# Shuijing725/CrowdNav_Prediction_AttnGraph

Hardware: NVIDIA H100
Metric: env_steps_per_s_ppo_rollout (higher is better)
Workload: dtype f32

## Files before the change

### crowdnav_prediction_attngraph_b200/csrc/cn_gemm_tc.cu

```cuda
#include "cn_gemm_tc.h"

__global__ void cn_split_f16_kernel(const float* __restrict__ src, float scale, __half* __restrict__ hi,
                                    __half* __restrict__ lo, size_t count) {
  const size_t i = (size_t)blockIdx.x * blockDim.x + threadIdx.x;
  if (i >= count) return;
  const float x = fminf(fmaxf(src[i] * scale, -65504.0f), 65504.0f);
  const __half h = __float2half_rn(x);
  hi[i] = h;
  lo[i] = __float2half_rn(x - __half2float(h));
}

namespace {

typedef CUresult (*EncodeFn)(CUtensorMap*, CUtensorMapDataType, cuuint32_t, void*, const cuuint64_t*, const cuuint64_t*,
                             const cuuint32_t*, const cuuint32_t*, CUtensorMapInterleave, CUtensorMapSwizzle,
                             CUtensorMapL2promotion, CUtensorMapFloatOOBfill);

EncodeFn get_encode() {
  static EncodeFn fn = nullptr;
  if (!fn) {
    void* sym = nullptr;
    cudaDriverEntryPointQueryResult qres;
    if (cudaGetDriverEntryPoint("cuTensorMapEncodeTiled", &sym, cudaEnableDefault, &qres) == cudaSuccess &&
        qres == cudaDriverEntryPointSuccess)
// ... 61 lines not shown
  cuuint64_t gstride[1] = {(cuuint64_t)pitch * esize};
  cuuint32_t box[2] = {(cuuint32_t)(128 / esize), 64};
  cuuint32_t estr[2] = {1, 1};
  CUresult r = enc(&s->map, esize == 4 ? CU_TENSOR_MAP_DATA_TYPE_FLOAT32 : CU_TENSOR_MAP_DATA_TYPE_FLOAT16, 2,
                   const_cast<void*>(ptr), gdim, gstride, box, estr, CU_TENSOR_MAP_INTERLEAVE_NONE,
                   CU_TENSOR_MAP_SWIZZLE_128B, CU_TENSOR_MAP_L2_PROMOTION_NONE, CU_TENSOR_MAP_FLOAT_OOB_FILL_NONE);
  if (r != CUDA_SUCCESS) return cn_set_error("cuTensorMapEncodeTiled(store) failed (%d) rows=%d cols=%d", (int)r, rows, cols);
  s->rows = rows; s->cols = cols;
  return 0;
}

int tc_alloc(CnLaunchCtx* c, TcMat& t, int rows, int K, int box_rows, int box_k) {
  int rc = halloc16(c, &t.hi, (size_t)rows * K);
  if (!rc) rc = halloc16(c, &t.lo, (size_t)rows * K);
  t.pitch = K; t.box_k = box_k;
  if (!rc) rc = make_map(&t.mh, t.hi, rows, K, box_rows, K, box_k);
  if (!rc) rc = make_map(&t.ml, t.lo, rows, K, box_rows, K, box_k);
  if (!rc) rc = tc_store_maps(t, rows, K);
  return rc;
}

int tc_view(TcMat& v, const TcMat& src, int col0, int rows, int K, int box_rows) {
  v.hi = src.hi + col0; v.lo = src.lo + col0; v.pitch = src.pitch; v.box_k = src.box_k;
  int rc = make_map(&v.mh, v.hi, rows, K, box_rows, src.pitch, src.box_k);
  if (!rc) rc = make_map(&v.ml, v.lo, rows, K, box_rows, src.pitch, src.box_k);
  if (!rc) rc = tc_store_maps(v, rows, K);
  return rc;
}

void split16(CnLaunchCtx* c, cudaStream_t st, const float* src, float scale, __half* hi, __half* lo, size_t count) {
  cn_split_f16_kernel<<<(unsigned)((count + 255) / 256), 256, 0, st>>>(src, scale, hi, lo, count);
  c->launches += 1;
}

int tc_set_attrs() {
  cudaError_t e = cudaSuccess;
  for (int act = CN_ACT_NONE; act <= CN_ACT_TANH; ++act)
    for (int out = TC_OUT_F32; out <= TC_OUT_BOTH; ++out) {
      if (e == cudaSuccess)
        e = cudaFuncSetAttribute(tc_kernel<256>(act, out), cudaFuncAttributeMaxDynamicSharedMemorySize, TcCfg<256>::kSmemBytes);
      if (e == cudaSuccess)
        e = cudaFuncSetAttribute(tc_kernel<64>(act, out), cudaFuncAttributeMaxDynamicSharedMemorySize, TcCfg<64>::kSmemBytes);
    }
  if (e == cudaSuccess)
    e = cudaFuncSetAttribute(cn_gemm_tc_kernel<64, true>, cudaFuncAttributeMaxDynamicSharedMemorySize, TcCfg<64>::kSmemBytes);
  if (e == cudaSuccess)
    e = cudaFuncSetAttribute(cn_gemm_tc_kernel<256, false, CN_ACT_NONE, TC_OUT_GRU>,
                             cudaFuncAttributeMaxDynamicSharedMemorySize, TcCfg<256>::kSmemBytes);
  if (e != cudaSuccess) return cn_set_error("cudaFuncSetAttribute(tc): %s", cudaGetErrorString(e));
  return 0;
}

void gemm_tc(CnLaunchCtx* c, cudaStream_t st, const TcMat& A, const TcMat& B, int M, int N, int K, int bn, const float* bias,
             int act, const TcOut& o, const int* m_ptr, int act_lo, int act_hi, const int* m0_ptr) {
  TcEpilogue ep;
  memset(&ep, 0, sizeof(ep));
  ep.bias = bias; ep.inv_scale = 1.0f / 64.0f; ep.act = act; ep.act_lo = act_lo; ep.act_hi = act_hi;
  ep.c32 = o.c32; ep.ldc = o.ldc; ep.out_hi = o.oh; ep.out_lo = o.ol; ep.ldh = o.ldh; ep.m_ptr = m_ptr; ep.m0_ptr = m0_ptr;
  {
    static const int nostore = (getenv("CN_DBG_NOSTORE") && getenv("CN_DBG_NOSTORE")[0] == '1') ? 1 : 0;
    ep.dbg_nostore = nostore;
  }
  if (A.box_k != tc_box_k(bn) || B.box_k != tc_box_k(bn)) {
    if (!c->launch_error) {
      c->launch_error = true;
      cn_set_error("gemm_tc in stage '%s': operand boxes %d / %d wide, the BN = %d instance loads %d",
                   c->cur_stage ? c->cur_stage : "?", A.box_k, B.box_k, bn, tc_box_k(bn));
    }
    return;
  }
  const int out_kind = (o.c32 ? TC_OUT_F32 : 0) | (o.oh ? TC_OUT_F16 : 0);
  if (act < CN_ACT_NONE || act > CN_ACT_TANH || !out_kind) {
    if (!c->launch_error) {
      c->launch_error = true;
      cn_set_error("gemm_tc in stage '%s': activation %d / no output", c->cur_stage ? c->cur_stage : "?", act);
    }
    return;
  }
#ifdef CN_GEMM_TRACE
  ep.trace = g_tc_trace; ep.trace_cap = g_tc_trace_cap;
#endif
  static const CUtensorMap no_map = {};
  const CUtensorMap *mc = &no_map, *mh = &no_map, *ml = &no_map;
  if (bn == 256) {
    auto fits = [&](const TcStoreMap* s) { return s && s->rows == M && s->cols == N; };
    const bool ok = (!o.c32 || fits(o.sc)) && (!o.oh || (fits(o.sh) && fits(o.sl)));
    if (!ok) {
      if (!c->launch_error) {
        c->launch_error = true;
        cn_set_error("gemm_tc in stage '%s': a BN = 256 output needs a TMA store map of [%d x %d] (16-byte-aligned "
                     "base, row pitch a multiple of 16 bytes)", c->cur_stage ? c->cur_stage : "?", M, N);
      }
      return;
    }
    if (o.c32) mc = &o.sc->map;
    if (o.oh) { mh = &o.sh->map; ml = &o.sl->map; }
  }
  const int tiles = (N / bn) * ((M + TC_BM - 1) / TC_BM);
  dim3 grid(tiles < c->num_sms ? tiles : c->num_sms);
  if (bn == 256)
    launch_k(c, tc_kernel<256>(act, out_kind), grid, dim3(TC_THREADS), TcCfg<256>::kSmemBytes, st, A.mh, A.ml, B.mh, B.ml, M, N, K, ep,
             *mc, *mh, *ml);
  else
    launch_k(c, tc_kernel<64>(act, out_kind), grid, dim3(TC_THREADS), TcCfg<64>::kSmemBytes, st, A.mh, A.ml, B.mh, B.ml, M, N, K, ep,
             *mc, *mh, *ml);
}

void gemm_tc_gru(CnLaunchCtx* c, cudaStream_t st, const TcMat& A, const TcMat& B, int M, const float* bias,
                 const float* h_in, const float* mask, float* h_out, int group, int pitch, int off, __half* oh, __half* ol,
                 int ldh) {
  const int N = 4 * 256, K = 64 + 256;
// ... 102 lines not shown
```

### crowdnav_prediction_attngraph_b200/csrc/cn_gemm_tc.cuh

```cuda
#pragma once
#include <cuda.h>
#include <cuda_fp16.h>
#include <cuda_runtime.h>
#include <stdint.h>

#include "cn_launch.cuh"

#define TC_BM 128
#define TC_BK 64
#define TC_CONSUMER_WARPS 8
#define TC_THREADS (128 + 32 * TC_CONSUMER_WARPS)

template <int BN>
struct TcCfg {
  static constexpr int kBK = (BN >= 256) ? 32 : TC_BK;
  static constexpr int kSwizzle = 2 * kBK;
  static constexpr int kStages = 4;
  static constexpr int kATile = TC_BM * kBK * 2;
  static constexpr int kBTile = BN * kBK * 2;
  static constexpr int kStageBytes = 2 * kATile + 2 * kBTile;
  static constexpr int kStoreBoxes = (BN >= 256) ? 2 : 0;
  static constexpr int kBoxBytes = 64 * 128;
  static constexpr int kStagingBytes = 2 * kStoreBoxes * kBoxBytes;
  static constexpr int kSmemBytes = kStages * kStageBytes + kStagingBytes + 256  + 1024 ;
};

struct TcEpilogue {
  const float* bias;
  float inv_scale;
  int act;
  int act_lo, act_hi;
  float* c32;
  int ldc;
  __half* out_hi;
  __half* out_lo;
  int ldh;
  const int* m_ptr;
  int dbg_nostore;
  const int* m0_ptr;
  const float* inv_scale_a;
  const float* inv_scale_b;
  int ksplit;
  const float* gru_h;
  const float* gru_mask;
  int gru_group, gru_pitch, gru_off;
#ifdef CN_GEMM_TRACE
  unsigned long long* trace;
  int trace_cap;
#endif
};

#ifdef CN_GEMM_TRACE
#define TC_TRACE_REC 7
#define TC_TRACE_WAIT_CLK 100
#endif

enum { TC_OUT_F32 = 1, TC_OUT_F16 = 2, TC_OUT_BOTH = 3, TC_OUT_GRU = 4 };

#ifdef CN_GEMM_TRACE
#define TC_TRACE(...) __VA_ARGS__
#else
#define TC_TRACE(...)
#endif

namespace tc {

__device__ __forceinline__ uint32_t smem_u32(const void* p) { return (uint32_t)__cvta_generic_to_shared(p); }

__device__ __forceinline__ void mbar_init(uint32_t bar, uint32_t count) {
  asm volatile("mbarrier.init.shared::cta.b64 [%0], %1;" ::"r"(bar), "r"(count));
}
__device__ __forceinline__ void mbar_expect_tx(uint32_t bar, uint32_t bytes) {
  asm volatile("mbarrier.arrive.expect_tx.shared::cta.b64 _, [%0], %1;" ::"r"(bar), "r"(bytes) : "memory");
}
__device__ __forceinline__ void mbar_arrive(uint32_t bar) {
  asm volatile("mbarrier.arrive.shared::cta.b64 _, [%0];" ::"r"(bar) : "memory");
}
__device__ __forceinline__ void mbar_wait(uint32_t bar, uint32_t parity) {
  uint32_t ok;
  do {
    asm volatile(
        "{\n"
        ".reg .pred p;\n"
        "mbarrier.try_wait.parity.shared::cta.b64 p, [%1], %2;\n"
        "selp.u32 %0, 1, 0, p;\n"
        "}\n" : "=r"(ok) : "r"(bar), "r"(parity) : "memory");
  } while (!ok);
}
#ifdef CN_GEMM_TRACE
__device__ __forceinline__ uint32_t mbar_wait_polls(uint32_t bar, uint32_t parity) {
  uint32_t ok, n = 0;
  while (true) {
// ... 351 lines not shown
  constexpr int TC_STAGE_BYTES = TcCfg<BN>::kStageBytes;
  constexpr bool kTmaStore = !PROMOTE && BN == 256 && OUT != TC_OUT_GRU;
  static_assert(OUT != TC_OUT_GRU || (BN == 256 && !PROMOTE), "the GRU epilogue reads four 64-column gate blocks");
  static_assert(!PROMOTE || BK == 64, "PROMOTE sums 64-wide k-blocks");
  static_assert(!kTmaStore || TcCfg<BN>::kStoreBoxes > 0, "BN = 256 stages its output");
  extern __shared__ uint8_t tc_smem_raw[];
  const uint32_t raw = tc::smem_u32(tc_smem_raw);
  const uint32_t base = (raw + 1023u) & ~1023u;
  const uint32_t staging = base + TC_STAGES * TC_STAGE_BYTES;
  const uint32_t bar_base = staging + TcCfg<BN>::kStagingBytes;
  const uint32_t bar_full = bar_base, bar_empty = bar_base + 64;

  const int warp = threadIdx.x >> 5, lane = threadIdx.x & 31, wg = warp >> 2;
  const int num_kb = K / BK;

  if (threadIdx.x == 0) {
    for (int s = 0; s < TC_STAGES; ++s) {
      tc::mbar_init(bar_full + 8 * s, 1);
      tc::mbar_init(bar_empty + 8 * s, TC_CONSUMER_WARPS);
    }
    asm volatile("fence.mbarrier_init.release.cluster;" ::: "memory");
    asm volatile("prefetch.tensormap [%0];" ::"l"(&map_ahi) : "memory");
    asm volatile("prefetch.tensormap [%0];" ::"l"(&map_alo) : "memory");
    asm volatile("prefetch.tensormap [%0];" ::"l"(&map_bhi) : "memory");
    asm volatile("prefetch.tensormap [%0];" ::"l"(&map_blo) : "memory");
    if constexpr (kTmaStore) {
      if constexpr ((OUT & TC_OUT_F32) != 0) asm volatile("prefetch.tensormap [%0];" ::"l"(&map_c) : "memory");
      if constexpr ((OUT & TC_OUT_F16) != 0) {
        asm volatile("prefetch.tensormap [%0];" ::"l"(&map_oh) : "memory");
        asm volatile("prefetch.tensormap [%0];" ::"l"(&map_ol) : "memory");
      }
    }
  }
  __syncthreads();
  cn_pdl_wait();
  const int m_ext = M;
  if (ep.m_ptr) { const int mc = *ep.m_ptr; M = mc < M ? mc : M; }
  int m_lo = ep.m0_ptr ? *ep.m0_ptr : 0;
  if (m_lo > M) m_lo = M;
  const int n_ntiles = N / BN;
  const int n_mn = ((M - m_lo + TC_BM - 1) / TC_BM) * n_ntiles;
  const int ksplit = (PROMOTE && ep.ksplit > 1) ? ep.ksplit : 1;
  const int kb_per = (num_kb + ksplit - 1) / ksplit;
  const int n_tiles = n_mn * ksplit;

  if (wg == 0) {
    tc::setmaxnreg_dec<40>();
    if (threadIdx.x == 0) {
      uint32_t it = 0;
      for (int tile = blockIdx.x; tile < n_tiles; tile += gridDim.x) {
        const int mn = tile % n_mn, ks = tile / n_mn;
        const int m0 = m_lo + (mn / n_ntiles) * TC_BM, n0 = (mn % n_ntiles) * BN;
        const int kb0 = ks * kb_per, kb1 = (kb0 + kb_per < num_kb) ? kb0 + kb_per : num_kb;
        for (int kb = kb0; kb < kb1; ++kb, ++it) {
          const uint32_t s = it % TC_STAGES, ph = (it / TC_STAGES) & 1u;
          tc::mbar_wait(bar_empty + 8 * s, ph ^ 1u);
          const uint32_t full = bar_full + 8 * s;
          tc::mbar_expect_tx(full, TC_STAGE_BYTES);
          const uint32_t st = base + s * TC_STAGE_BYTES;
          tc::tma_load_2d(st, &map_ahi, full, kb * BK, m0);
          tc::tma_load_2d(st + TC_A_TILE_BYTES, &map_alo, full, kb * BK, m0);
          tc::tma_load_2d(st + 2 * TC_A_TILE_BYTES, &map_bhi, full, kb * BK, n0);
          tc::tma_load_2d(st + 2 * TC_A_TILE_BYTES + TC_B_TILE_BYTES, &map_blo, full, kb * BK, n0);
        }
      }
    }
    return;
  }
  tc::setmaxnreg_inc<232>();
  float inv_scale = ep.inv_scale;
  if (ep.inv_scale_a) inv_scale *= __ldg(ep.inv_scale_a);
  if (ep.inv_scale_b) inv_scale *= __ldg(ep.inv_scale_b);
  const int half = wg - 1;
  const int wr = 16 * (warp & 3) + (lane >> 2);
  const int cq = 2 * (lane & 3);
  uint32_t it = 0;
  TcStaging sg;
  sg.base = staging + half * TcCfg<BN>::kStoreBoxes * TcCfg<BN>::kBoxBytes;
  sg.box = 0; sg.leader = (threadIdx.x & 127) == 0; sg.bar_id = wg;
  TC_TRACE(sg.waits = 0; sg.wait_clk = 0;)
  TC_TRACE(const bool tr = ep.trace && warp == 4 && lane == 0; int tr_n = 0;)
  for (int tile = blockIdx.x; tile < n_tiles; tile += gridDim.x) {
    const int mn = tile % n_mn, ks = tile / n_mn;
    const int m0 = m_lo + (mn / n_ntiles) * TC_BM, n0 = (mn % n_ntiles) * BN;
    const int kb0 = ks * kb_per, kb1 = (kb0 + kb_per < num_kb) ? kb0 + kb_per : num_kb;
    TC_TRACE(const uint64_t t_tile = tc::globaltimer(); uint64_t t_first = 0; uint32_t polls = 0;)
    float acc[BN / 2];
    float sum[PROMOTE ? BN / 2 : 1];
    if constexpr (PROMOTE) {
#pragma unroll
      for (int i = 0; i < BN / 2; ++i) sum[i] = 0.0f;
    }
    uint32_t prev = 0;
    for (int kb = kb0; kb < kb1; ++kb, ++it) {
      const uint32_t s = it % TC_STAGES, ph = (it / TC_STAGES) & 1u;
#ifdef CN_GEMM_TRACE
      polls += tc::mbar_wait_polls(bar_full + 8 * s, ph);
      if (kb == kb0) t_first = tc::globaltimer();
#else
      tc::mbar_wait(bar_full + 8 * s, ph);
#endif
      const uint32_t st = base + s * TC_STAGE_BYTES;
      const uint32_t a_hi = st + half * (TC_A_TILE_BYTES / 2), a_lo = a_hi + TC_A_TILE_BYTES,
                     b_hi = st + 2 * TC_A_TILE_BYTES, b_lo = b_hi + TC_B_TILE_BYTES;
      tc::fence_regs(acc);
      tc::wgmma_fence();
#pragma unroll
      for (int k = 0; k < BK / 16; ++k) {
        const uint32_t koff = k * 32;
        const uint64_t dah = tc::make_desc<SW>(a_hi + koff), dal = tc::make_desc<SW>(a_lo + koff);
        const uint64_t dbh = tc::make_desc<SW>(b_hi + koff), dbl = tc::make_desc<SW>(b_lo + koff);
        const bool first = k == 0 && (PROMOTE || kb == kb0);
        tc::wgmma_f16<BN>(acc, dah, dbh, first ? 0u : 1u);
        tc::wgmma_f16<BN>(acc, dah, dbl, 1u);
// ... 95 lines not shown
```

### crowdnav_prediction_attngraph_b200/csrc/cn_gemm_tc.h

```cpp
#pragma once
#include <cuda.h>
#include <cuda_fp16.h>
#include <cuda_runtime.h>
#include <stdint.h>

#include "cn_gemm_tc.cuh"
#include "cn_launch.cuh"

struct TcStoreMap {
  CUtensorMap map;
  int rows = 0, cols = 0;
};

struct TcMat {
  __half *hi = nullptr, *lo = nullptr;
  CUtensorMap mh, ml;
  int pitch = 0;
  int box_k = 0;
  TcStoreMap sh, sl;
};

struct TcOut {
  float* c32 = nullptr; int ldc = 0;
  __half *oh = nullptr, *ol = nullptr; int ldh = 0;
  const TcStoreMap *sc = nullptr, *sh = nullptr, *sl = nullptr;
};
inline TcOut out32(float* c, int ldc, const TcStoreMap* sc = nullptr) { TcOut o; o.c32 = c; o.ldc = ldc; o.sc = sc; return o; }
inline TcOut out16(const TcMat& t) { TcOut o; o.oh = t.hi; o.ol = t.lo; o.ldh = t.pitch; o.sh = &t.sh; o.sl = &t.sl; return o; }
inline TcOut out_both(float* c, int ldc, const TcMat& t) { TcOut o = out16(t); o.c32 = c; o.ldc = ldc; return o; }

inline int tc_box_k(int bn) { return bn == 256 ? TcCfg<256>::kBK : TcCfg<64>::kBK; }

inline bool tma_store_ok(const void* ptr, size_t pitch_bytes) { return ((uintptr_t)ptr % 16) == 0 && pitch_bytes % 16 == 0; }

int make_map(CUtensorMap* map, const __half* ptr, int rows, int K, int box_rows, int pitch, int box_k = TC_BK);
int make_store_map(TcStoreMap* s, const void* ptr, int esize, int rows, int cols, int pitch);
int tc_alloc(CnLaunchCtx* c, TcMat& t, int rows, int K, int box_rows, int box_k);
int tc_view(TcMat& v, const TcMat& src, int col0, int rows, int K, int box_rows);
void split16(CnLaunchCtx* c, cudaStream_t st, const float* src, float scale, __half* hi, __half* lo, size_t count);
int tc_set_attrs();

void gemm_tc(CnLaunchCtx* c, cudaStream_t st, const TcMat& A, const TcMat& B, int M, int N, int K, int bn, const float* bias,
             int act, const TcOut& o, const int* m_ptr = nullptr, int act_lo = 0, int act_hi = 1 << 30,
             const int* m0_ptr = nullptr);

void gemm_tc_gru(CnLaunchCtx* c, cudaStream_t st, const TcMat& A, const TcMat& B, int M, const float* bias,
                 const float* h_in, const float* mask, float* h_out, int group, int pitch, int off, __half* oh, __half* ol,
                 int ldh);

int gemm_tc_promote(int num_sms, cudaStream_t st, const __half* ahi, const __half* alo, int a_rows, int a_pitch,
                    const __half* bhi, const __half* blo, int b_rows, int b_pitch, int Kd, float* C, int ldc,
                    const float* bias, int act, const float* inv_a, const float* inv_b, int ksplit);
```

### crowdnav_prediction_attngraph_b200/csrc/cn_policy.cu

```cuda
#include <cuda_runtime.h>
#include <stdio.h>
#include <stdlib.h>
#include <string.h>
#include <map>
#include <string>
#include <vector>

#include "../../include/crowdnav_b200.h"
#include "cn_host_util.h"
#include "cn_gemm_tc.h"
#include "cn_launch.cuh"
#include "cn_policy_kernels.cuh"
#include "cn_qkv_attn.cuh"

struct cn_policy {
  cn_policy_config cfg;
  int N, H, Win, M;
  CnLaunchCtx lc;
  bool fuse_qkv;
  TcMat tWqkvH;
  CUtensorMap qa_ah, qa_al, qa_bh, qa_bl;
  float* bqkvH = nullptr;
  int* tile_tab = nullptr;
  cudaEvent_t ev_tiles;
  void (*attn_kernel)(const float*, const int*, const int*, const int*, const int*, float*, __half*, __half*);
  int attn_warps;
  int qkv_chunks;
  bool finalized;
  std::map<std::string, std::vector<float>> host;
  size_t ws_allocs;
  float *W1, *b1, *W2, *b2, *Wqkv, *bqkv, *Wos, *bos;
  float *Wr, *br, *Wet, *bet, *WsT, *bs, *Wa, *ba, *Wih, *bih, *Whh, *bhh, *Wo, *bo;
  float *Woac, *boac;
  float *Wac1, *bac1, *Wa2, *ba2, *Wc2, *bc2, *wv_, *bv, *Wm, *bm, *logstd;
  TcMat tW2, tWqkv, tWos, tWet, tWsT, tWa, tWih, tWhh, tWo, tWac1, tWoac, tWa2, tWc2;
  TcMat tE1, tE2, tAo;
  TcMat tRs, tT1, tTe, tWv, tH0, tH1, tOut, tAc1, tA1, tC1;
  cudaStream_t st2, st3;
  cudaEvent_t ev_fork, ev_join, ev_fork2, ev_join2, ev_fork3, ev_join3;
  bool profile;
  std::vector<cudaEvent_t> ev;
  int *row_start, *row_env, *mc;
  float *x16, *e1, *e2, *qkv, *ao, *sout, *xr, *rs, *t1, *u, *wv, *h0, *gi, *gh, *outb, *ac1, *a2, *c2;
  TcStoreMap qkv_st, sout_st;
};

void cn_hr_attention_dense(CnLaunchCtx* c, cudaStream_t st, const float* s_out, const float* u, const float* te, int ldte,
                           int te_off, const float* b_s, int env_pitch, int env_off, int N, int H, float* wv,
                           __half* wv_hi, __half* wv_lo, int ldwh) {
  launch_k(c, cn_hr_attention_kernel<true>, dim3((N + 3) / 4), dim3(128), 0, st, s_out, u, te, ldte, te_off, b_s,
           (const int*)nullptr, env_pitch, env_off, N, H, wv, wv_hi, wv_lo, ldwh);
}

namespace {

int upload(cn_policy* p, float** dst, const std::vector<float>& src) {
  int rc = palloc(&p->lc, dst, src.size());
  if (rc) return rc;
  cudaError_t err = cudaMemcpy(*dst, src.data(), src.size() * sizeof(float), cudaMemcpyHostToDevice);
  if (err != cudaSuccess) return cn_set_error("H2D param: %s", cudaGetErrorString(err));
  return 0;
}

const std::vector<float>* get(cn_policy* p, const char* key, size_t count) {
  auto it = p->host.find(key);
  if (it == p->host.end()) { cn_set_error("cn_policy_finalize: parameter '%s' was not set", key); return nullptr; }
  if (it->second.size() != count) {
    cn_set_error("cn_policy_finalize: parameter '%s' has %zu elements, expected %zu", key, it->second.size(), count);
    return nullptr;
  }
  return &it->second;
}

void gemm(cn_policy* p, cudaStream_t st, const float* A, int lda, const float* W, int ldw, const float* bias,
          float* C, int ldc, int M, int N, int K, int act, int act_lo = 0, int act_hi = 1 << 30,
          const int* m_ptr = nullptr, __half* oh = nullptr, __half* ol = nullptr) {
  dim3 grid((N + CN_GEMM_BN - 1) / CN_GEMM_BN, (M + CN_GEMM_BM - 1) / CN_GEMM_BM);
  launch_k(&p->lc, cn_gemm_f32_kernel, grid, dim3(256), 0, st, A, lda, W, ldw, bias, C, ldc, M, N, K, act, act_lo, act_hi, m_ptr, oh, ol);
}

const char* kStageNames[] = {"pack_inputs", "embed1_gemm", "embed2_gemm", "qkv_gemm", "hh_attention",
                             "outproj_spatial_gemm", "robot_branch_join", "hr_attention", "gru", "actor_critic_heads"};
const int kNumStages = sizeof(kStageNames) / sizeof(kStageNames[0]);

inline void mark(cn_policy* p, cudaStream_t st, int i) {
  p->lc.cur_stage = i < kNumStages ? kStageNames[i] : "end";
  if (p->profile) cudaEventRecord(p->ev[i], st);
}

}

extern "C" {

int cn_policy_profile(cn_policy* p, int enable) {
  if (!p) return cn_set_error("cn_policy_profile: null argument");
  cudaSetDevice(p->cfg.device);
// ... 20 lines not shown
  if (!cfg || !out) return cn_set_error("cn_policy_create: null argument");
  *out = nullptr;
  if (cfg->num_envs <= 0 || cfg->human_num <= 0 || cfg->human_num > 128 || cfg->input_size <= 0 || cfg->input_size > 16)
    return cn_set_error("cn_policy_create: unsupported dims N=%d H=%d input=%d", cfg->num_envs, cfg->human_num,
                        cfg->input_size);
  int ndev = 0;
  cudaError_t err = cudaGetDeviceCount(&ndev);
  if (err != cudaSuccess || ndev == 0)
    return cn_set_error("cn_policy_create: no CUDA device (%s); this engine has no CPU fallback",
                        err == cudaSuccess ? "device count 0" : cudaGetErrorString(err));
  if (cfg->device < 0 || cfg->device >= ndev) return cn_set_error("cn_policy_create: bad device %d", cfg->device);
  cudaSetDevice(cfg->device);
  cn_policy* p = new cn_policy();
  p->cfg = *cfg;
  p->N = cfg->num_envs; p->H = cfg->human_num; p->Win = cfg->input_size; p->M = p->N * p->H;
  p->finalized = false; p->profile = false;
  cn_launch_init(&p->lc, cfg->device);
  {
    const char* qc = getenv("CN_QKV_CHUNKS");
    p->qkv_chunks = (qc && qc[0] == '2') ? 2 : 1;
    const char* ar = getenv("CN_ATTN_R");
    const int attn_r = ar ? atoi(ar) : 1;
    p->attn_kernel = attn_r == 1 ? cn_hh_attention_kernel<1, 4, 4> : (attn_r == 4 ? cn_hh_attention_kernel<4, 2, 2> : cn_hh_attention_kernel<2, 4, 4>);
    p->attn_warps = attn_r == 4 ? 2 : 4;
    const char* fq = getenv("CN_FUSE_QKV");
    p->fuse_qkv = cfg->gemm_mode == 1 && p->qkv_chunks == 1 && (fq && fq[0] == '1') && p->N <= QA_MAX_ENVS && p->H <= 128;
  }
  cudaEventCreateWithFlags(&p->ev_tiles, cudaEventDisableTiming);
  cudaStreamCreateWithFlags(&p->st2, cudaStreamNonBlocking);
  cudaStreamCreateWithFlags(&p->st3, cudaStreamNonBlocking);
  cudaEventCreateWithFlags(&p->ev_fork3, cudaEventDisableTiming);
  cudaEventCreateWithFlags(&p->ev_join3, cudaEventDisableTiming);
  cudaEventCreateWithFlags(&p->ev_fork, cudaEventDisableTiming);
  cudaEventCreateWithFlags(&p->ev_join, cudaEventDisableTiming);
  cudaEventCreateWithFlags(&p->ev_fork2, cudaEventDisableTiming);
  cudaEventCreateWithFlags(&p->ev_join2, cudaEventDisableTiming);
  const size_t M = (size_t)p->M, N = (size_t)p->N;
  const int Mi = p->M, Ni = p->N;
  int rc = 0;
#define WS(name, count) if (!rc) rc = palloc(&p->lc, &p->name, (count))
  {
    float* q = nullptr;
    if (!rc) rc = palloc(&p->lc, &q, N + 2);
    p->row_start = reinterpret_cast<int*>(q);
    if (!rc) rc = palloc(&p->lc, &q, 4);
    p->mc = reinterpret_cast<int*>(q);
    if (!rc) rc = palloc(&p->lc, &q, M + 1);
    p->row_env = reinterpret_cast<int*>(q);
    if (!rc) rc = palloc(&p->lc, &q, 2 * N + 4);
    p->tile_tab = reinterpret_cast<int*>(q);
  }
  WS(x16, M * 16); WS(e1, M * 128); WS(e2, M * 512); WS(qkv, M * 1536); WS(ao, M * 512); WS(sout, M * 256);
  WS(xr, N * 16); WS(rs, N * 256); WS(t1, N * 128); WS(u, N * 256); WS(wv, N * 256); WS(h0, N * 128);
  WS(gi, N * 384); WS(gh, N * 384); WS(outb, N * 256); WS(ac1, N * 512); WS(a2, N * 256); WS(c2, N * 256);
#undef WS
  if (!rc && cfg->gemm_mode == 1) {
    rc = tc_alloc(&p->lc, p->tE1, Mi, 128, TC_BM, tc_box_k(256));
    if (!rc) rc = tc_alloc(&p->lc, p->tE2, Mi, 512, TC_BM, tc_box_k(256));
    if (!rc) rc = tc_alloc(&p->lc, p->tAo, Mi, 512, TC_BM, tc_box_k(256));
    if (!rc) rc = tc_alloc(&p->lc, p->tRs, Ni, 256, TC_BM, tc_box_k(64));
    if (!rc) rc = tc_alloc(&p->lc, p->tT1, Ni, 128, TC_BM, tc_box_k(64));
    if (!rc) rc = tc_view(p->tTe, p->tT1, 64, Ni, 64, TC_BM);
    if (!rc) rc = tc_alloc(&p->lc, p->tWv, Ni, 256, TC_BM, tc_box_k(64));
    if (!rc) rc = tc_alloc(&p->lc, p->tH0, Ni, 128, TC_BM, tc_box_k(64));
    if (!rc) rc = tc_alloc(&p->lc, p->tH1, Ni, 128, TC_BM, tc_box_k(64));
    if (!rc) rc = tc_alloc(&p->lc, p->tOut, Ni, 256, TC_BM, tc_box_k(64));
    if (!rc) rc = tc_alloc(&p->lc, p->tAc1, Ni, 512, TC_BM, tc_box_k(64));
    if (!rc) rc = tc_view(p->tA1, p->tAc1, 0, Ni, 256, TC_BM);
    if (!rc) rc = tc_view(p->tC1, p->tAc1, 256, Ni, 256, TC_BM);
    if (!rc) rc = make_store_map(&p->qkv_st, p->qkv, 4, Mi, 1536, 1536);
    if (!rc) rc = make_store_map(&p->sout_st, p->sout, 4, Mi, 256, 256);
    if (!rc) rc = tc_set_attrs();
    if (!rc) {
      err = cudaFuncSetAttribute(cn_qkv_attn_kernel, cudaFuncAttributeMaxDynamicSharedMemorySize, QA_SMEM_BYTES);
      if (err != cudaSuccess) rc = cn_set_error("cudaFuncSetAttribute(qkv_attn): %s", cudaGetErrorString(err));
    }
  }
  if (rc) { cn_policy_destroy(p); return rc; }
  p->ws_allocs = p->lc.allocs.size();
  *out = p;
  return 0;
}

int cn_policy_destroy(cn_policy* p) {
  if (!p) return 0;
  cudaSetDevice(p->cfg.device);
  cn_launch_free(&p->lc);
  for (auto& e : p->ev) cudaEventDestroy(e);
  if (p->st2) {
    cudaStreamDestroy(p->st2);
    cudaStreamDestroy(p->st3); cudaEventDestroy(p->ev_fork3); cudaEventDestroy(p->ev_join3); cudaEventDestroy(p->ev_tiles);
    cudaEventDestroy(p->ev_fork); cudaEventDestroy(p->ev_join); cudaEventDestroy(p->ev_fork2); cudaEventDestroy(p->ev_join2);
  }
  delete p;
  return 0;
}

int cn_policy_set_param(cn_policy* p, const char* key, const float* h_data, size_t count) {
  if (!p || !key || !h_data) return cn_set_error("cn_policy_set_param: null argument");
  p->host[key] = std::vector<float>(h_data, h_data + count);
  p->finalized = false;
  return 0;
}

int cn_policy_finalize(cn_policy* p, void* stream) {
  if (!p) return cn_set_error("cn_policy_finalize: null argument");
  cudaSetDevice(p->cfg.device);
  cudaStream_t st = (cudaStream_t)stream;
  const int Win = p->Win;
#define GET(var, key, count) const std::vector<float>* var = get(p, key, (count)); if (!var) return 1
  GET(w1, "base.spatial_attn.embedding_layer.0.weight", (size_t)128 * Win);
  GET(b1, "base.spatial_attn.embedding_layer.0.bias", 128);
  GET(w2, "base.spatial_attn.embedding_layer.2.weight", (size_t)512 * 128);
  GET(b2, "base.spatial_attn.embedding_layer.2.bias", 512);
  GET(wq, "base.spatial_attn.q_linear.weight", (size_t)512 * 512);
  GET(bq, "base.spatial_attn.q_linear.bias", 512);
  GET(wk, "base.spatial_attn.k_linear.weight", (size_t)512 * 512);
  GET(bk, "base.spatial_attn.k_linear.bias", 512);
  GET(wvv, "base.spatial_attn.v_linear.weight", (size_t)512 * 512);
  GET(bvv, "base.spatial_attn.v_linear.bias", 512);
  GET(win, "base.spatial_attn.multihead_attn.in_proj_weight", (size_t)1536 * 512);
  GET(bin, "base.spatial_attn.multihead_attn.in_proj_bias", 1536);
// ... 5 lines not shown
  GET(br, "base.robot_linear.0.bias", 256);
  GET(wt, "base.attn.temporal_edge_layer.0.weight", (size_t)64 * 256);
  GET(bt, "base.attn.temporal_edge_layer.0.bias", 64);
  GET(ws, "base.attn.spatial_edge_layer.0.weight", (size_t)64 * 256);
  GET(bs, "base.attn.spatial_edge_layer.0.bias", 64);
  GET(we, "base.humanNodeRNN.encoder_linear.weight", (size_t)64 * 256);
  GET(be, "base.humanNodeRNN.encoder_linear.bias", 64);
  GET(wa, "base.humanNodeRNN.edge_attention_embed.weight", (size_t)64 * 256);
  GET(ba, "base.humanNodeRNN.edge_attention_embed.bias", 64);
  GET(wih, "base.humanNodeRNN.gru.weight_ih_l0", (size_t)384 * 128);
  GET(whh, "base.humanNodeRNN.gru.weight_hh_l0", (size_t)384 * 128);
  GET(bih, "base.humanNodeRNN.gru.bias_ih_l0", 384);
  GET(bhh, "base.humanNodeRNN.gru.bias_hh_l0", 384);
  GET(wo, "base.humanNodeRNN.output_linear.weight", (size_t)256 * 128);
  GET(bo, "base.humanNodeRNN.output_linear.bias", 256);
  GET(wa0, "base.actor.0.weight", (size_t)256 * 256);
  GET(ba0, "base.actor.0.bias", 256);
  GET(wa2, "base.actor.2.weight", (size_t)256 * 256);
  GET(ba2, "base.actor.2.bias", 256);
  GET(wc0, "base.critic.0.weight", (size_t)256 * 256);
  GET(bc0, "base.critic.0.bias", 256);
  GET(wc2, "base.critic.2.weight", (size_t)256 * 256);
  GET(bc2, "base.critic.2.bias", 256);
  GET(wcl, "base.critic_linear.weight", 256);
  GET(bcl, "base.critic_linear.bias", 1);
  GET(wm, "dist.fc_mean.weight", (size_t)2 * 256);
  GET(bm, "dist.fc_mean.bias", 2);
  GET(ls, "dist.logstd._bias", 2);
#undef GET
  cudaStreamSynchronize(st);
  for (size_t i = p->ws_allocs; i < p->lc.allocs.size(); ++i) cudaFree(p->lc.allocs[i]);
  p->lc.allocs.resize(p->ws_allocs);
  int rc = 0;
  auto pad_k = [](const std::vector<float>& w, int rows, int k, int kp) {
    std::vector<float> o((size_t)rows * kp, 0.0f);
    for (int r = 0; r < rows; ++r) for (int c = 0; c < k; ++c) o[(size_t)r * kp + c] = w[(size_t)r * k + c];
    return o;
  };
  auto cat = [](const std::vector<float>& a, const std::vector<float>& b) {
    std::vector<float> o(a); o.insert(o.end(), b.begin(), b.end()); return o;
  };
#define UP(dst, vec) if (!rc) rc = upload(p, &p->dst, (vec))
  UP(W1, pad_k(*w1, 128, Win, 16)); UP(b1, *b1); UP(W2, *w2); UP(b2, *b2);
  UP(Wr, pad_k(*wr, 256, 9, 16)); UP(br, *br);
  UP(Wet, cat(*we, *wt)); UP(bet, cat(*be, *bt));
  {
    std::vector<float> wst((size_t)256 * 64);
    for (int r = 0; r < 64; ++r) for (int c = 0; c < 256; ++c) wst[(size_t)c * 64 + r] = (*ws)[(size_t)r * 256 + c];
    UP(WsT, wst);
  }
  UP(bs, *bs); UP(Wa, *wa); UP(ba, *ba); UP(Wih, *wih); UP(bih, *bih); UP(Whh, *whh); UP(bhh, *bhh);
  UP(Wo, *wo); UP(bo, *bo);
  UP(Wac1, cat(*wa0, *wc0)); UP(bac1, cat(*ba0, *bc0));
  UP(Wa2, *wa2); UP(ba2, *ba2); UP(Wc2, *wc2); UP(bc2, *bc2);
  UP(wv_, *wcl); UP(bv, *bcl); UP(Wm, *wm); UP(bm, *bm); UP(logstd, *ls);
#undef UP
  float *d_win = nullptr, *d_bin = nullptr, *d_wl[3] = {nullptr, nullptr, nullptr}, *d_bl[3] = {nullptr, nullptr, nullptr};
  float *d_wout = nullptr, *d_bout = nullptr, *d_wsl = nullptr, *d_bsl = nullptr;
  if (!rc) rc = upload(p, &d_win, *win);
  if (!rc) rc = upload(p, &d_bin, *bin);
  const std::vector<float>* wl[3] = {wq, wk, wvv};
  const std::vector<float>* bl[3] = {bq, bk, bvv};
  for (int i = 0; i < 3 && !rc; ++i) { rc = upload(p, &d_wl[i], *wl[i]); if (!rc) rc = upload(p, &d_bl[i], *bl[i]); }
  if (!rc) rc = upload(p, &d_wout, *wout);
  if (!rc) rc = upload(p, &d_bout, *bout);
  if (!rc) rc = upload(p, &d_wsl, *wsl);
  if (!rc) rc = upload(p, &d_bsl, *bsl);
  if (!rc) rc = palloc(&p->lc, &p->Wqkv, (size_t)1536 * 512);
  if (!rc) rc = palloc(&p->lc, &p->bqkv, 1536);
  if (!rc) rc = palloc(&p->lc, &p->Wos, (size_t)256 * 512);
  if (!rc) rc = palloc(&p->lc, &p->bos, 256);
  if (!rc) rc = palloc(&p->lc, &p->Woac, (size_t)512 * 128);
  if (!rc) rc = palloc(&p->lc, &p->boac, 512);
  if (rc) return rc;
  for (int i = 0; i < 3; ++i) {
    cn_fold_mm_kernel<<<dim3(4, 512), 128, 0, st>>>(d_win + (size_t)i * 512 * 512, d_wl[i],
                                                     p->Wqkv + (size_t)i * 512 * 512, 512, 512, 512);
    cn_fold_mv_kernel<<<4, 128, 0, st>>>(d_win + (size_t)i * 512 * 512, d_bl[i], d_bin + i * 512, p->bqkv + i * 512, 512, 512);
  }
  cn_fold_mm_kernel<<<dim3(4, 256), 128, 0, st>>>(d_wsl, d_wout, p->Wos, 256, 512, 512);
  cn_fold_mv_kernel<<<2, 128, 0, st>>>(d_wsl, d_bout, d_bsl, p->bos, 256, 512);
  cn_fold_mm_kernel<<<dim3(1, 512), 128, 0, st>>>(p->Wac1, p->Wo, p->Woac, 512, 128, 256);
  cn_fold_mv_kernel<<<4, 128, 0, st>>>(p->Wac1, p->bo, p->bac1, p->boac, 512, 256);
  if (p->cfg.gemm_mode == 1) {
    struct { float* src; TcMat* t; int rows, k, bn; } tw[13] = {
        {p->Woac, &p->tWoac, 512, 128, 64},
        {p->W2, &p->tW2, 512, 128, 256},    {p->Wqkv, &p->tWqkv, 1536, 512, 256}, {p->Wos, &p->tWos, 256, 512, 256},
        {p->Wet, &p->tWet, 128, 256, 64},   {p->WsT, &p->tWsT, 256, 64, 64},      {p->Wa, &p->tWa, 64, 256, 64},
        {p->Wih, &p->tWih, 384, 128, 64},   {p->Whh, &p->tWhh, 384, 128, 64},     {p->Wo, &p->tWo, 256, 128, 64},
        {p->Wac1, &p->tWac1, 512, 256, 64}, {p->Wa2, &p->tWa2, 256, 256, 64},     {p->Wc2, &p->tWc2, 256, 256, 64}};
    for (auto& t : tw) {
      rc = tc_alloc(&p->lc, *t.t, t.rows, t.k, t.bn, tc_box_k(t.bn));
      if (rc) return rc;
      split16(&p->lc, st, t.src, 64.0f, t.t->hi, t.t->lo, (size_t)t.rows * t.k);
    }
    if (p->fuse_qkv) {
      float* wh = nullptr;
      rc = palloc(&p->lc, &wh, (size_t)1536 * 512);
      if (!rc) rc = palloc(&p->lc, &p->bqkvH, 1536);
      if (!rc) rc = tc_alloc(&p->lc, p->tWqkvH, 1536, 512, QA_BN, QA_BK);
      if (!rc) rc = make_map(&p->qa_bh, p->tWqkvH.hi, 1536, 512, QA_BN, 512, QA_BK);
      if (!rc) rc = make_map(&p->qa_bl, p->tWqkvH.lo, 1536, 512, QA_BN, 512, QA_BK);
      if (!rc) rc = make_map(&p->qa_ah, p->tE2.hi, p->M, 512, TC_BM, 512, QA_BK);
      if (!rc) rc = make_map(&p->qa_al, p->tE2.lo, p->M, 512, TC_BM, 512, QA_BK);
      if (rc) return rc;
      cn_head_major_kernel<<<1536, 128, 0, st>>>(p->Wqkv, p->bqkv, wh, p->bqkvH);
      split16(&p->lc, st, wh, 64.0f, p->tWqkvH.hi, p->tWqkvH.lo, (size_t)1536 * 512);
    }
  }
  cudaError_t err = cudaStreamSynchronize(st);
  if (err != cudaSuccess) return cn_set_error("cn_policy_finalize: %s", cudaGetErrorString(err));
  p->finalized = true;
  return 0;
}

int cn_policy_act(cn_policy* p, const cn_act_ptrs* d, void* stream) {
  if (!p || !d) return cn_set_error("cn_policy_act: null argument");
  if (!p->finalized) return cn_set_error("cn_policy_act: call cn_policy_finalize after setting parameters");
  if (!d->robot_node || !d->temporal_edges || !d->spatial_edges || !d->detected_human_num || !d->h_in || !d->masks ||
      !d->value || !d->action || !d->log_prob || !d->h_out)
    return cn_set_error("cn_policy_act: missing input/output pointer");
  CnDeviceGuard guard(p->cfg.device);
  cudaStream_t st = (cudaStream_t)stream;
  const int N = p->N, H = p->H, M = p->M;
  const bool tcm = p->cfg.gemm_mode == 1;
  const int* mc = p->mc;
  const int ALL = 1 << 30;
  mark(p, st, 0);
  {
    launch_k(&p->lc, cn_row_offsets_kernel, dim3(1), dim3(1024), 0, st, d->detected_human_num, N, H, p->row_start, p->mc);
    const int total = (!tcm && M * 16 > N * 128) ? M * 16 : N * 128;
    launch_k(&p->lc, cn_pack_inputs_kernel, dim3((total + 255) / 256), dim3(256), 0, st, d->spatial_edges, p->Win, H, N, p->row_start, p->row_env,
                                                               tcm ? nullptr : p->x16,
                                                               d->temporal_edges, d->robot_node, d->h_in, d->masks, p->xr,
                                                               p->h0, tcm ? p->tH0.hi : nullptr, tcm ? p->tH0.lo : nullptr);
  }
  cudaStream_t s2 = p->st2;
  cudaEventRecord(p->ev_fork, st);
  cudaStreamWaitEvent(s2, p->ev_fork, 0);
  if (p->fuse_qkv) {
    cn_qkv_tiles_kernel<<<1, 1024, 0, s2>>>(p->row_start, N, p->tile_tab);
    p->lc.launches += 1;
    cudaEventRecord(p->ev_tiles, s2);
// ... 25 lines not shown
    __half* al = p->tAo.lo;
    if (p->fuse_qkv) {
      cudaStreamWaitEvent(st, p->ev_tiles, 0);
      launch_k(&p->lc, cn_qkv_attn_kernel, dim3(p->lc.num_sms), dim3(QA_THREADS), QA_SMEM_BYTES, st, p->qa_ah, p->qa_al, p->qa_bh,
               p->qa_bl, p->bqkvH, 1.0f / 64.0f, p->tile_tab, p->row_start, p->row_env, ah, al,
               getenv("CN_QA_DBG") ? atoi(getenv("CN_QA_DBG")) : 0);
      mark(p, st, 4);
    } else if (p->qkv_chunks == 1) {
      gemm_tc(&p->lc, st, p->tE2, p->tWqkv, M, 1536, 512, 256, p->bqkv, CN_ACT_NONE, out32(p->qkv, 1536, &p->qkv_st), mc);
      mark(p, st, 4);
      launch_k(&p->lc, p->attn_kernel, dim3(p->lc.num_sms * 64 / p->attn_warps), dim3(p->attn_warps * 32), 0, st, p->qkv, p->row_start, p->row_env, mc, nullptr,
                                                                             nullptr, ah, al);
    } else {
    gemm_tc(&p->lc, st, p->tE2, p->tWqkv, M, 1536, 512, 256, p->bqkv, CN_ACT_NONE, out32(p->qkv, 1536, &p->qkv_st), mid);
    cudaEventRecord(p->ev_fork3, st);
    cudaStreamWaitEvent(p->st3, p->ev_fork3, 0);
    launch_k(&p->lc, p->attn_kernel, dim3(p->lc.num_sms * 32 / p->attn_warps), dim3(p->attn_warps * 32), 0, p->st3, p->qkv, p->row_start, p->row_env, mid, nullptr,
                                                                              nullptr, ah, al);
    cudaEventRecord(p->ev_join3, p->st3);
    gemm_tc(&p->lc, st, p->tE2, p->tWqkv, M, 1536, 512, 256, p->bqkv, CN_ACT_NONE, out32(p->qkv, 1536, &p->qkv_st), mc, 0, 1 << 30, mid);
    mark(p, st, 4);
    launch_k(&p->lc, p->attn_kernel, dim3(p->lc.num_sms * 64 / p->attn_warps), dim3(p->attn_warps * 32), 0, st, p->qkv, p->row_start, p->row_env, mc, mid, nullptr,
                                                                           ah, al);
    cudaStreamWaitEvent(st, p->ev_join3, 0);
    }
  } else {
    gemm(p, st, p->e2, 512, p->Wqkv, 512, p->bqkv, p->qkv, 1536, M, 1536, 512, CN_ACT_NONE, 0, ALL, mc);
    mark(p, st, 4);
    launch_k(&p->lc, p->attn_kernel, dim3(p->lc.num_sms * 64 / p->attn_warps), dim3(p->attn_warps * 32), 0, st, p->qkv, p->row_start, p->row_env, p->mc, nullptr,
                                                                           p->ao, nullptr, nullptr);
  }
  mark(p, st, 5);
  if (tcm) gemm_tc(&p->lc, st, p->tAo, p->tWos, M, 256, 512, 256, p->bos, CN_ACT_RELU, out32(p->sout, 256, &p->sout_st), mc);
  else gemm(p, st, p->ao, 512, p->Wos, 512, p->bos, p->sout, 256, M, 256, 512, CN_ACT_RELU, 0, ALL, mc);
  mark(p, st, 6);
  cudaStreamWaitEvent(st, p->ev_join, 0);
  mark(p, st, 7);
  launch_k(&p->lc, cn_hr_attention_kernel<false>, dim3((N + 3) / 4), dim3(128), 0, st, p->sout, p->u, p->t1, 128, 64, p->bs, p->row_start, 0, 0,
                                                      N, H, p->wv, tcm ? p->tWv.hi : nullptr, tcm ? p->tWv.lo : nullptr, 256);
  mark(p, st, 8);
  if (tcm) {
    TcOut o; o.oh = p->tT1.hi + 64; o.ol = p->tT1.lo + 64; o.ldh = 128;
    gemm_tc(&p->lc, st, p->tWv, p->tWa, N, 64, 256, 64, p->ba, CN_ACT_RELU, o);
    gemm_tc(&p->lc, st, p->tT1, p->tWih, N, 384, 128, 64, p->bih, CN_ACT_NONE, out32(p->gi, 384));
  } else {
    gemm(p, st, p->wv, 256, p->Wa, 256, p->ba, p->t1 + 64, 128, N, 64, 256, CN_ACT_RELU);
    gemm(p, st, p->t1, 128, p->Wih, 128, p->bih, p->gi, 384, N, 384, 128, CN_ACT_NONE);
  }
  launch_k(&p->lc, cn_gru_gate_kernel, dim3((N * 128 + 255) / 256), dim3(256), 0, st, p->gi, p->gh, p->h0, N, d->h_out, tcm ? p->tH1.hi : nullptr,
                                                            tcm ? p->tH1.lo : nullptr);
  mark(p, st, 9);
  if (tcm) {
    gemm_tc(&p->lc, st, p->tH1, p->tWoac, N, 512, 128, 64, p->boac, CN_ACT_TANH, out16(p->tAc1));
    cudaEventRecord(p->ev_fork2, st);
    cudaStreamWaitEvent(s2, p->ev_fork2, 0);
    gemm_tc(&p->lc, s2, p->tC1, p->tWc2, N, 256, 256, 64, p->bc2, CN_ACT_TANH, out32(p->c2, 256));
    cudaEventRecord(p->ev_join2, s2);
    gemm_tc(&p->lc, st, p->tA1, p->tWa2, N, 256, 256, 64, p->ba2, CN_ACT_TANH, out32(p->a2, 256));
  } else {
    gemm(p, st, d->h_out, 128, p->Woac, 128, p->boac, p->ac1, 512, N, 512, 128, CN_ACT_TANH);
    cudaEventRecord(p->ev_fork2, st);
    cudaStreamWaitEvent(s2, p->ev_fork2, 0);
    gemm(p, s2, p->ac1 + 256, 512, p->Wc2, 256, p->bc2, p->c2, 256, N, 256, 256, CN_ACT_TANH);
    cudaEventRecord(p->ev_join2, s2);
    gemm(p, st, p->ac1, 512, p->Wa2, 256, p->ba2, p->a2, 256, N, 256, 256, CN_ACT_TANH);
  }
  cudaStreamWaitEvent(st, p->ev_join2, 0);
  launch_k(&p->lc, cn_heads_kernel, dim3((N + 3) / 4), dim3(128), 0, st, p->a2, 256, p->c2, 256, p->wv_, p->bv, p->Wm, p->bm, p->logstd, d->noise, N,
                                               d->value, d->action, d->log_prob, d->action_mean);
  mark(p, st, kNumStages);
  cudaError_t err = cudaGetLastError();
  if (p->lc.launch_error) { p->lc.launch_error = false; return 1; }
  if (err != cudaSuccess) return cn_set_error("cn_policy_act launch: %s", cudaGetErrorString(err));
  return 0;
}

int64_t cn_policy_launch_count(cn_policy* p) { return p ? p->lc.launches : 0; }

int64_t cn_policy_last_rows(cn_policy* p) {
  if (!p) return -1;
  cudaSetDevice(p->cfg.device);
  int v = 0;
  if (cudaDeviceSynchronize() != cudaSuccess || cudaMemcpy(&v, p->mc, sizeof(int), cudaMemcpyDeviceToHost) != cudaSuccess)
    return -1;
  return v;
}

int cn_internal_policy_buffer(cn_policy* p, const char* name, void** ptr, void** ptr_lo, int* rows, int* cols, int* ld,
                              int* kind) {
  if (!p || !name || !ptr || !ptr_lo || !rows || !cols || !ld || !kind)
    return cn_set_error("cn_internal_policy_buffer: null argument");
  const bool tcm = p->cfg.gemm_mode == 1;
  const int N = p->N, M = p->M;
  const std::string s(name);
  *ptr_lo = nullptr;
  auto f32 = [&](const float* q, int r, int c, int l) { *ptr = (void*)q; *rows = r; *cols = c; *ld = l; *kind = 0; return 0; };
  auto i32 = [&](const int* q, int r) { *ptr = (void*)q; *rows = r; *cols = 1; *ld = 1; *kind = 2; return 0; };
  auto f16 = [&](const TcMat& t, int r, int c) {
    *ptr = t.hi; *ptr_lo = t.lo; *rows = r; *cols = c; *ld = t.pitch; *kind = 1; return 0;
  };
  if (s == "row_start") return i32(p->row_start, N + 1);
  if (s == "row_env") return i32(p->row_env, M);
  if (s == "mc") return i32(p->mc, 1);
  if (s == "e1") return tcm ? f16(p->tE1, M, 128) : f32(p->e1, M, 128, 128);
  if (s == "e2") return tcm ? f16(p->tE2, M, 512) : f32(p->e2, M, 512, 512);
  if (s == "qkv") {
    if (p->fuse_qkv) return cn_set_error("cn_internal_policy_buffer: 'qkv' is never written by the fused QKV-attention kernel");
    return f32(p->qkv, M, 1536, 1536);
  }
  if (s == "ao") return tcm ? f16(p->tAo, M, 512) : f32(p->ao, M, 512, 512);
  if (s == "sout") return f32(p->sout, M, 256, 256);
  if (s == "rs") return tcm ? f16(p->tRs, N, 256) : f32(p->rs, N, 256, 256);
  if (s == "t1") return tcm ? f16(p->tT1, N, 128) : f32(p->t1, N, 128, 128);
  if (s == "u") return f32(p->u, N, 256, 256);
  if (s == "wv") return tcm ? f16(p->tWv, N, 256) : f32(p->wv, N, 256, 256);
  if (s == "h0") return tcm ? f16(p->tH0, N, 128) : f32(p->h0, N, 128, 128);
  if (s == "gi") return f32(p->gi, N, 384, 384);
  if (s == "gh") return f32(p->gh, N, 384, 384);
  if (s == "h1") {
    if (!tcm) return cn_set_error("cn_internal_policy_buffer: 'h1' exists in gemm_mode 1 only (gemm_mode 0 reads h_out)");
    return f16(p->tH1, N, 128);
  }
  if (s == "ac1") return tcm ? f16(p->tAc1, N, 512) : f32(p->ac1, N, 512, 512);
  if (s == "a2") return f32(p->a2, N, 256, 256);
  if (s == "c2") return f32(p->c2, N, 256, 256);
  if (tcm && s == "t1.f32") return f32(p->t1, N, 128, 128);
  if (tcm && s == "wv.f32") return f32(p->wv, N, 256, 256);
  if (tcm && s == "h0.f32") return f32(p->h0, N, 128, 128);
  if (!p->finalized && (s == "Wqkv" || s == "bqkv" || s == "Wos" || s == "bos" || s == "Woac" || s == "boac"))
    return cn_set_error("cn_internal_policy_buffer: '%s' needs cn_policy_finalize first", name);
  if (s == "Wqkv") return f32(p->Wqkv, 1536, 512, 512);
  if (s == "bqkv") return f32(p->bqkv, 1536, 1, 1);
  if (s == "Wos") return f32(p->Wos, 256, 512, 512);
  if (s == "bos") return f32(p->bos, 256, 1, 1);
  if (s == "Woac") return f32(p->Woac, 512, 128, 128);
  if (s == "boac") return f32(p->boac, 512, 1, 1);
  return cn_set_error("cn_internal_policy_buffer: unknown buffer '%s' (gemm_mode %d)", name, p->cfg.gemm_mode);
}

}
```

Before: 6.880 million.

## Fuse actor and critic second-layer GEMMs into one grouped tensor-core launch

The separate actor and critic 256x256 GEMMs, previously run on two forked streams, become one N=512 GEMM over concatenated weights. A new per-column-group A offset lets each 256-wide output group read its own half of the shared activation buffer. Outputs are interleaved into a single 512-pitch buffer read by the heads kernel. This removes one launch plus the stream fork/join events, but gives up concurrency between the two streams.

Result: no change. 6.851 million (median of 6 runs) (-0.4%).

```diff
diff --git a/crowdnav_prediction_attngraph_b200/csrc/cn_gemm_tc.cu b/crowdnav_prediction_attngraph_b200/csrc/cn_gemm_tc.cu
--- a/crowdnav_prediction_attngraph_b200/csrc/cn_gemm_tc.cu
+++ b/crowdnav_prediction_attngraph_b200/csrc/cn_gemm_tc.cu
@@ -137,11 +137,20 @@
 }
 
 void gemm_tc(CnLaunchCtx* c, cudaStream_t st, const TcMat& A, const TcMat& B, int M, int N, int K, int bn, const float* bias,
-             int act, const TcOut& o, const int* m_ptr, int act_lo, int act_hi, const int* m0_ptr) {
+             int act, const TcOut& o, const int* m_ptr, int act_lo, int act_hi, const int* m0_ptr, int a_group_n) {
   TcEpilogue ep;
   memset(&ep, 0, sizeof(ep));
   ep.bias = bias; ep.inv_scale = 1.0f / 64.0f; ep.act = act; ep.act_lo = act_lo; ep.act_hi = act_hi;
   ep.c32 = o.c32; ep.ldc = o.ldc; ep.out_hi = o.oh; ep.out_lo = o.ol; ep.ldh = o.ldh; ep.m_ptr = m_ptr; ep.m0_ptr = m0_ptr;
+  ep.a_group_n = a_group_n;
+  if (a_group_n < 0 || a_group_n % bn) {
+    if (!c->launch_error) {
+      c->launch_error = true;
+      cn_set_error("gemm_tc in stage '%s': column group %d is not a multiple of the tile width %d",
+                   c->cur_stage ? c->cur_stage : "?", a_group_n, bn);
+    }
+    return;
+  }
   {
     static const int nostore = (getenv("CN_DBG_NOSTORE") && getenv("CN_DBG_NOSTORE")[0] == '1') ? 1 : 0;
     ep.dbg_nostore = nostore;
diff --git a/crowdnav_prediction_attngraph_b200/csrc/cn_gemm_tc.cuh b/crowdnav_prediction_attngraph_b200/csrc/cn_gemm_tc.cuh
--- a/crowdnav_prediction_attngraph_b200/csrc/cn_gemm_tc.cuh
+++ b/crowdnav_prediction_attngraph_b200/csrc/cn_gemm_tc.cuh
@@ -38,6 +38,7 @@
   const int* m_ptr;
   int dbg_nostore;
   const int* m0_ptr;
+  int a_group_n;
   const float* inv_scale_a;
   const float* inv_scale_b;
   int ksplit;
@@ -495,14 +496,15 @@
         const int mn = tile % n_mn, ks = tile / n_mn;
         const int m0 = m_lo + (mn / n_ntiles) * TC_BM, n0 = (mn % n_ntiles) * BN;
         const int kb0 = ks * kb_per, kb1 = (kb0 + kb_per < num_kb) ? kb0 + kb_per : num_kb;
+        const int ka = ep.a_group_n ? (n0 / ep.a_group_n) * K : 0;
         for (int kb = kb0; kb < kb1; ++kb, ++it) {
           const uint32_t s = it % TC_STAGES, ph = (it / TC_STAGES) & 1u;
           tc::mbar_wait(bar_empty + 8 * s, ph ^ 1u);
           const uint32_t full = bar_full + 8 * s;
           tc::mbar_expect_tx(full, TC_STAGE_BYTES);
           const uint32_t st = base + s * TC_STAGE_BYTES;
-          tc::tma_load_2d(st, &map_ahi, full, kb * BK, m0);
-          tc::tma_load_2d(st + TC_A_TILE_BYTES, &map_alo, full, kb * BK, m0);
+          tc::tma_load_2d(st, &map_ahi, full, ka + kb * BK, m0);
+          tc::tma_load_2d(st + TC_A_TILE_BYTES, &map_alo, full, ka + kb * BK, m0);
           tc::tma_load_2d(st + 2 * TC_A_TILE_BYTES, &map_bhi, full, kb * BK, n0);
           tc::tma_load_2d(st + 2 * TC_A_TILE_BYTES + TC_B_TILE_BYTES, &map_blo, full, kb * BK, n0);
         }
diff --git a/crowdnav_prediction_attngraph_b200/csrc/cn_gemm_tc.h b/crowdnav_prediction_attngraph_b200/csrc/cn_gemm_tc.h
--- a/crowdnav_prediction_attngraph_b200/csrc/cn_gemm_tc.h
+++ b/crowdnav_prediction_attngraph_b200/csrc/cn_gemm_tc.h
@@ -42,7 +42,7 @@
 
 void gemm_tc(CnLaunchCtx* c, cudaStream_t st, const TcMat& A, const TcMat& B, int M, int N, int K, int bn, const float* bias,
              int act, const TcOut& o, const int* m_ptr = nullptr, int act_lo = 0, int act_hi = 1 << 30,
-             const int* m0_ptr = nullptr);
+             const int* m0_ptr = nullptr, int a_group_n = 0);
 
 void gemm_tc_gru(CnLaunchCtx* c, cudaStream_t st, const TcMat& A, const TcMat& B, int M, const float* bias,
                  const float* h_in, const float* mask, float* h_out, int group, int pitch, int off, __half* oh, __half* ol,
diff --git a/crowdnav_prediction_attngraph_b200/csrc/cn_policy.cu b/crowdnav_prediction_attngraph_b200/csrc/cn_policy.cu
--- a/crowdnav_prediction_attngraph_b200/csrc/cn_policy.cu
+++ b/crowdnav_prediction_attngraph_b200/csrc/cn_policy.cu
@@ -32,16 +32,17 @@
   float *W1, *b1, *W2, *b2, *Wqkv, *bqkv, *Wos, *bos;
   float *Wr, *br, *Wet, *bet, *WsT, *bs, *Wa, *ba, *Wih, *bih, *Whh, *bhh, *Wo, *bo;
   float *Woac, *boac;
-  float *Wac1, *bac1, *Wa2, *ba2, *Wc2, *bc2, *wv_, *bv, *Wm, *bm, *logstd;
-  TcMat tW2, tWqkv, tWos, tWet, tWsT, tWa, tWih, tWhh, tWo, tWac1, tWoac, tWa2, tWc2;
+  float *Wac1, *bac1, *Wac2, *bac2, *wv_, *bv, *Wm, *bm, *logstd;
+  TcMat tW2, tWqkv, tWos, tWet, tWsT, tWa, tWih, tWhh, tWo, tWac1, tWoac, tWac2;
   TcMat tE1, tE2, tAo;
-  TcMat tRs, tT1, tTe, tWv, tH0, tH1, tOut, tAc1, tA1, tC1;
+  TcMat tRs, tT1, tTe, tWv, tH0, tH1, tOut, tAc1;
   cudaStream_t st2, st3;
   cudaEvent_t ev_fork, ev_join, ev_fork2, ev_join2, ev_fork3, ev_join3;
   bool profile;
   std::vector<cudaEvent_t> ev;
   int *row_start, *row_env, *mc;
-  float *x16, *e1, *e2, *qkv, *ao, *sout, *xr, *rs, *t1, *u, *wv, *h0, *gi, *gh, *outb, *ac1, *a2, *c2;
+  float *x16, *e1, *e2, *qkv, *ao, *sout, *xr, *rs, *t1, *u, *wv, *h0, *gi, *gh, *outb, *ac1;
+  float *a2, *c2;
   TcStoreMap qkv_st, sout_st;
 };
 
@@ -168,8 +169,10 @@
   }
   WS(x16, M * 16); WS(e1, M * 128); WS(e2, M * 512); WS(qkv, M * 1536); WS(ao, M * 512); WS(sout, M * 256);
   WS(xr, N * 16); WS(rs, N * 256); WS(t1, N * 128); WS(u, N * 256); WS(wv, N * 256); WS(h0, N * 128);
-  WS(gi, N * 384); WS(gh, N * 384); WS(outb, N * 256); WS(ac1, N * 512); WS(a2, N * 256); WS(c2, N * 256);
+  WS(gi, N * 384); WS(gh, N * 384); WS(outb, N * 256); WS(ac1, N * 512);
+  WS(a2, N * 512 + 256);
 #undef WS
+  p->c2 = p->a2 + 256;
   if (!rc && cfg->gemm_mode == 1) {
     rc = tc_alloc(&p->lc, p->tE1, Mi, 128, TC_BM, tc_box_k(256));
     if (!rc) rc = tc_alloc(&p->lc, p->tE2, Mi, 512, TC_BM, tc_box_k(256));
@@ -182,8 +185,6 @@
     if (!rc) rc = tc_alloc(&p->lc, p->tH1, Ni, 128, TC_BM, tc_box_k(64));
     if (!rc) rc = tc_alloc(&p->lc, p->tOut, Ni, 256, TC_BM, tc_box_k(64));
     if (!rc) rc = tc_alloc(&p->lc, p->tAc1, Ni, 512, TC_BM, tc_box_k(64));
-    if (!rc) rc = tc_view(p->tA1, p->tAc1, 0, Ni, 256, TC_BM);
-    if (!rc) rc = tc_view(p->tC1, p->tAc1, 256, Ni, 256, TC_BM);
     if (!rc) rc = make_store_map(&p->qkv_st, p->qkv, 4, Mi, 1536, 1536);
     if (!rc) rc = make_store_map(&p->sout_st, p->sout, 4, Mi, 256, 256);
     if (!rc) rc = tc_set_attrs();
@@ -295,7 +296,7 @@
   UP(bs, *bs); UP(Wa, *wa); UP(ba, *ba); UP(Wih, *wih); UP(bih, *bih); UP(Whh, *whh); UP(bhh, *bhh);
   UP(Wo, *wo); UP(bo, *bo);
   UP(Wac1, cat(*wa0, *wc0)); UP(bac1, cat(*ba0, *bc0));
-  UP(Wa2, *wa2); UP(ba2, *ba2); UP(Wc2, *wc2); UP(bc2, *bc2);
+  UP(Wac2, cat(*wa2, *wc2)); UP(bac2, cat(*ba2, *bc2));
   UP(wv_, *wcl); UP(bv, *bcl); UP(Wm, *wm); UP(bm, *bm); UP(logstd, *ls);
 #undef UP
   float *d_win = nullptr, *d_bin = nullptr, *d_wl[3] = {nullptr, nullptr, nullptr}, *d_bl[3] = {nullptr, nullptr, nullptr};
@@ -326,12 +327,12 @@
   cn_fold_mm_kernel<<<dim3(1, 512), 128, 0, st>>>(p->Wac1, p->Wo, p->Woac, 512, 128, 256);
   cn_fold_mv_kernel<<<4, 128, 0, st>>>(p->Wac1, p->bo, p->bac1, p->boac, 512, 256);
   if (p->cfg.gemm_mode == 1) {
-    struct { float* src; TcMat* t; int rows, k, bn; } tw[13] = {
+    struct { float* src; TcMat* t; int rows, k, bn; } tw[12] = {
         {p->Woac, &p->tWoac, 512, 128, 64},
         {p->W2, &p->tW2, 512, 128, 256},    {p->Wqkv, &p->tWqkv, 1536, 512, 256}, {p->Wos, &p->tWos, 256, 512, 256},
         {p->Wet, &p->tWet, 128, 256, 64},   {p->WsT, &p->tWsT, 256, 64, 64},      {p->Wa, &p->tWa, 64, 256, 64},
         {p->Wih, &p->tWih, 384, 128, 64},   {p->Whh, &p->tWhh, 384, 128, 64},     {p->Wo, &p->tWo, 256, 128, 64},
-        {p->Wac1, &p->tWac1, 512, 256, 64}, {p->Wa2, &p->tWa2, 256, 256, 64},     {p->Wc2, &p->tWc2, 256, 256, 64}};
+        {p->Wac1, &p->tWac1, 512, 256, 64}, {p->Wac2, &p->tWac2, 512, 256, 64}};
     for (auto& t : tw) {
       rc = tc_alloc(&p->lc, *t.t, t.rows, t.k, t.bn, tc_box_k(t.bn));
       if (rc) return rc;
@@ -463,21 +464,18 @@
   mark(p, st, 9);
   if (tcm) {
     gemm_tc(&p->lc, st, p->tH1, p->tWoac, N, 512, 128, 64, p->boac, CN_ACT_TANH, out16(p->tAc1));
-    cudaEventRecord(p->ev_fork2, st);
-    cudaStreamWaitEvent(s2, p->ev_fork2, 0);
-    gemm_tc(&p->lc, s2, p->tC1, p->tWc2, N, 256, 256, 64, p->bc2, CN_ACT_TANH, out32(p->c2, 256));
-    cudaEventRecord(p->ev_join2, s2);
-    gemm_tc(&p->lc, st, p->tA1, p->tWa2, N, 256, 256, 64, p->ba2, CN_ACT_TANH, out32(p->a2, 256));
+    gemm_tc(&p->lc, st, p->tAc1, p->tWac2, N, 512, 256, 64, p->bac2, CN_ACT_TANH, out32(p->a2, 512), nullptr, 0, 1 << 30,
+            nullptr, 256);
   } else {
     gemm(p, st, d->h_out, 128, p->Woac, 128, p->boac, p->ac1, 512, N, 512, 128, CN_ACT_TANH);
     cudaEventRecord(p->ev_fork2, st);
     cudaStreamWaitEvent(s2, p->ev_fork2, 0);
-    gemm(p, s2, p->ac1 + 256, 512, p->Wc2, 256, p->bc2, p->c2, 256, N, 256, 256, CN_ACT_TANH);
+    gemm(p, s2, p->ac1 + 256, 512, p->Wac2 + 256 * 256, 256, p->bac2 + 256, p->c2, 512, N, 256, 256, CN_ACT_TANH);
     cudaEventRecord(p->ev_join2, s2);
-    gemm(p, st, p->ac1, 512, p->Wa2, 256, p->ba2, p->a2, 256, N, 256, 256, CN_ACT_TANH);
-  }
-  cudaStreamWaitEvent(st, p->ev_join2, 0);
-  launch_k(&p->lc, cn_heads_kernel, dim3((N + 3) / 4), dim3(128), 0, st, p->a2, 256, p->c2, 256, p->wv_, p->bv, p->Wm, p->bm, p->logstd, d->noise, N,
+    gemm(p, st, p->ac1, 512, p->Wac2, 256, p->bac2, p->a2, 512, N, 256, 256, CN_ACT_TANH);
+    cudaStreamWaitEvent(st, p->ev_join2, 0);
+  }
+  launch_k(&p->lc, cn_heads_kernel, dim3((N + 3) / 4), dim3(128), 0, st, p->a2, 512, p->c2, 512, p->wv_, p->bv, p->Wm, p->bm, p->logstd, d->noise, N,
                                                d->value, d->action, d->log_prob, d->action_mean);
   mark(p, st, kNumStages);
   cudaError_t err = cudaGetLastError();
@@ -533,8 +531,8 @@
     return f16(p->tH1, N, 128);
   }
   if (s == "ac1") return tcm ? f16(p->tAc1, N, 512) : f32(p->ac1, N, 512, 512);
-  if (s == "a2") return f32(p->a2, N, 256, 256);
-  if (s == "c2") return f32(p->c2, N, 256, 256);
+  if (s == "a2") return f32(p->a2, N, 256, 512);
+  if (s == "c2") return f32(p->c2, N, 256, 512);
   if (tcm && s == "t1.f32") return f32(p->t1, N, 128, 128);
   if (tcm && s == "wv.f32") return f32(p->wv, N, 256, 256);
   if (tcm && s == "h0.f32") return f32(p->h0, N, 128, 128);
```
